# HenryHZY/VL-PET

Measured on AMD Instinct MI355X. Metric: multitask samples/sec (BART-base, r=96), higher is better.
Workload: dtype bf16

## Files before the change

vl-pet_amd/csrc/attn.hip:

```cpp
#include <cstdlib>
#include "common.h"
#include "kernels.h"
#include "attn_common.h"

#define AT_NW 4

__device__ __forceinline__ void stage_image(uint8_t* img, const __bf16* src, int64_t rs, int n_rows, int rows_pad, int tid, int nthreads) {
    const u32x4 z = {0u, 0u, 0u, 0u};
    for (int idx = tid; idx < rows_pad * 8; idx += nthreads) {
        const int row = idx >> 3, pc = idx & 7;
        u32x4 v = z;
        if (row < n_rows) v = __builtin_nontemporal_load(reinterpret_cast<const u32x4*>(src + (int64_t)row * rs + pc * 8));
        *reinterpret_cast<u32x4*>(img + (size_t)row * AT_ROW + pc * 16) = v;
    }
}
template <int NIMG, int MAXP>
__device__ __forceinline__ void stage_images(uint8_t* const* img, const __bf16* const* src, const int* n_rows, const int* rows_pad,
                                             const int64_t* rs, int tid, int nthreads) {
    u32x4 v[NIMG][MAXP];
#pragma unroll
    for (int g = 0; g < NIMG; ++g)
#pragma unroll
        for (int c = 0; c < MAXP; ++c) {
            const int idx = tid + c * nthreads, row = idx >> 3, pc = idx & 7;
            const int rr = row < n_rows[g] ? row : n_rows[g] - 1;
            v[g][c] = __builtin_nontemporal_load(reinterpret_cast<const u32x4*>(src[g] + (int64_t)rr * rs[g] + pc * 8));
        }
    const u32x4 z = {0u, 0u, 0u, 0u};
#pragma unroll
    for (int g = 0; g < NIMG; ++g)
#pragma unroll
        for (int c = 0; c < MAXP; ++c) {
            const int idx = tid + c * nthreads, row = idx >> 3, pc = idx & 7;
            if (row < rows_pad[g]) *reinterpret_cast<u32x4*>(img[g] + (size_t)row * AT_ROW + pc * 16) = row < n_rows[g] ? v[g][c] : z;
        }
}

#define AT_FW 2

struct AttnLds {
    __host__ __device__ static constexpr size_t fwd_wave_bytes(int Lkp) { return (size_t)Lkp * AT_ROW + (size_t)AT_STG + (size_t)Lkp * 4; }
    static size_t fwd_bytes(int Lkp) { return (size_t)AT_FW * fwd_wave_bytes(Lkp); }
    static size_t bwd_bytes(int Lqp, int Lkp) {
        return bwd_bytes_nw(Lqp, Lkp, AT_NW);
    }
    static size_t bwd_bytes_nw(int Lqp, int Lkp, int nw) {
        return (size_t)2 * (Lqp + Lkp) * AT_ROW + (size_t)nw * AT_STG + (size_t)Lqp * 12 + (size_t)Lkp * 4;
    }
};

__device__ __forceinline__ float key_bias(const AttnArgs& a, const uint8_t* km, int key) {
    return (key < a.Lk && (km == nullptr || km[key] != 0)) ? 0.f : -INFINITY;
}

template <int T, bool BIAS>
__global__ __launch_bounds__(AT_FW * 64, (T <= 2 ? 3 : 2)) void attn_fwd_kernel(AttnArgs a) {
    extern __shared__ __attribute__((aligned(16))) uint8_t smem[];
    const int tid = threadIdx.x, lane = tid & 63, wave = __builtin_amdgcn_readfirstlane(tid >> 6);
    const int bh = blockIdx.x * AT_FW + wave;
    if (bh >= a.B * a.H) return;
    const uint64_t seed = a.thr ? vlpet_eff_seed(a.seed, a.seed_ctr) : 0;
    const int b = bh / a.H, h = bh % a.H;
    const int m = lane & 31, hh = lane >> 5;
    constexpr int Lkp = 32 * T;
    const int64_t rs = (int64_t)a.H * 64, rq = a.ld_q, rk = a.ld_kv, rv = a.ld_v;
    const __bf16* qb_ = a.q + (int64_t)b * a.Lq * rq + h * 64;
    const __bf16* kb_ = a.k + (int64_t)b * a.Lk * rk + h * 64;
    const __bf16* vb_ = a.v + (int64_t)b * a.Lk * rv + h * 64;
    __bf16* ob_ = a.o + (int64_t)b * a.Lq * rs + h * 64;
    const uint8_t* km = a.key_mask ? a.key_mask + (int64_t)b * a.Lk : nullptr;
    uint8_t* Vs = smem + (size_t)wave * AttnLds::fwd_wave_bytes(Lkp);
    uint8_t* stg = Vs + (size_t)Lkp * AT_ROW;
    float* kval = reinterpret_cast<float*>(stg + AT_STG);
#pragma unroll
    for (int c = 0; c < (Lkp + 63) / 64; ++c)
        if (lane + 64 * c < Lkp) kval[lane + 64 * c] = key_bias(a, km, lane + 64 * c);
    const int coff = a.causal ? a.Lk - a.Lq : (1 << 20);

    bf16x8 kf[T][4];
#pragma unroll
    for (int t = 0; t < T; ++t) {
        const int j = 32 * t + m, jk = j < a.Lk ? j : a.Lk - 1;
#pragma unroll
        for (int ks = 0; ks < 4; ++ks) kf[t][ks] = *reinterpret_cast<const bf16x8*>(kb_ + (int64_t)jk * rk + 16 * ks + 8 * hh);
    }
    stage_image(Vs, vb_, rv, a.Lk, Lkp, lane, 64);

    const float sc2 = a.scale * AT_LOG2E;
    const int NQB = (a.Lq + 31) >> 5;
    for (int qb = 0; qb < NQB; ++qb) {
        const int i = 32 * qb + m;
        const int iq = i < a.Lq ? i : a.Lq - 1;
        bf16x8 qf[4];
#pragma unroll
        for (int ks = 0; ks < 4; ++ks) qf[ks] = *reinterpret_cast<const bf16x8*>(qb_ + (int64_t)iq * rq + 16 * ks + 8 * hh);
        f32x16 st[T];
#pragma unroll
        for (int t = 0; t < T; ++t) {
            if constexpr (BIAS) st[t] = bias_tile(a.bias + ((int64_t)h * (32 * NQB) + i) * Lkp + 32 * t + 4 * hh, 1.0f / a.scale);
            else st[t] = zero16();
#pragma unroll
            for (int ks = 0; ks < 4; ++ks) st[t] = mfma32(kf[t][ks], qf[ks], st[t]);
        }
        float mx = -INFINITY;
        const int ic = i + coff - 4 * hh;
#pragma unroll
        for (int t = 0; t < T; ++t) {
#pragma unroll
            for (int q4 = 0; q4 < 4; ++q4) {
                const f32x4 kv = *reinterpret_cast<const f32x4*>(kval + 32 * t + 8 * q4 + 4 * hh);
#pragma unroll
                for (int e = 0; e < 4; ++e) {
                    const int r = 4 * q4 + e;
                    float s = fmaf(st[t][r], sc2, kv[e]);
                    s = 32 * t + e + 8 * q4 > ic ? -INFINITY : s;
                    st[t][r] = s;
                    mx = fmaxf(mx, s);
                }
            }
        }
        mx = fmaxf(mx, __shfl_xor(mx, 32));
        if (mx == -INFINITY) mx = 0.f;
        float sum = 0.f;
#pragma unroll
        for (int t = 0; t < T; ++t) {
#pragma unroll
            for (int r = 0; r < 16; ++r) { const float p = fast_exp2(st[t][r] - mx); st[t][r] = p; sum += p; }
        }
        sum += __shfl_xor(sum, 32);
        const float inv = sum > 0.f ? 1.0f / sum : 0.f;
        if (hh == 0 && i < a.Lq) a.lse[((int64_t)b * a.H + h) * a.Lq + i] = sum > 0.f ? mx + log2f(sum) : INFINITY;
        const uint32_t rk = row_key(seed, ((int64_t)b * a.H + h) * a.Lq + iq);
        const float inv_keep = a.thr ? a.inv_keep : 1.0f;
        f32x16 ot0 = zero16(), ot1 = zero16();
#pragma unroll
        for (int t = 0; t < T; ++t) {
            if (a.keep_out != nullptr && a.thr != 0) {
#pragma unroll
                for (int r = 0; r < 16; ++r) {
                    const int key = 32 * t + (r & 3) + 8 * (r >> 2) + 4 * hh;
                    if (i < a.Lq && key < a.Lk)
                        a.keep_out[(((int64_t)b * a.H + h) * a.Lq + i) * a.Lk + key] = keep_elem(rk, key, a.thr) ? 1 : 0;
                }
            }
            const uint32_t kg0 = rk + (uint32_t)(32 * t + 4 * hh) * AT_GOLD;
#pragma unroll
            for (int r = 0; r < 16; ++r) {
                const int ir = (r & 3) + 8 * (r >> 2);
                const bool kp = hash_elem(kg0 + (uint32_t)ir * AT_GOLD) >= a.thr;
                st[t][r] = kp ? st[t][r] * inv * inv_keep : 0.f;
            }
#pragma unroll
            for (int u = 0; u < 2; ++u) {
                const bf16x8 pf = acc_frag(st[t], u);
                ot0 = mfma32(tr_acc_order(Vs, 32 * t + 16 * u, 0, lane), pf, ot0);
                ot1 = mfma32(tr_acc_order(Vs, 32 * t + 16 * u, 32, lane), pf, ot1);
            }
        }
        store_rows_T(stg, ot0, ot1, ob_, rs, 32 * qb, a.Lq, lane);
    }
}

enum { IMG_Q = 0, IMG_D = 1, IMG_K = 2, IMG_V = 3 };
struct BwdCtx {
    const float* rowt;
    const float* kval;
    int Lqp;
    float sc2, scale, inv_keep;
    uint32_t thr;
    int coff;
};
__device__ __forceinline__ BwdCtx bwd_ctx(const AttnArgs& a, const float* rowt, const float* kval, int Lqp) {
    BwdCtx c;
    c.rowt = rowt; c.kval = kval; c.Lqp = Lqp;
    c.sc2 = a.scale * AT_LOG2E; c.scale = a.scale; c.inv_keep = a.thr ? a.inv_keep : 1.0f; c.thr = a.thr;
    c.coff = a.causal ? a.Lk - a.Lq : (1 << 20);
    return c;
}

template <class R, bool BIAS>
__device__ __forceinline__ void bwd_k_unit(const AttnArgs& a, const BwdCtx& c, const R& rd0, int t, int NQB, int Lqp, int Lkp, int h, int lane,
                                           f32x16& dv0, f32x16& dv1, f32x16& dk0, f32x16& dk1) {
    const int m = lane & 31, hh = lane >> 5;
    const int key = 32 * t + m;
    const float kb = c.kval[key];
    const uint32_t kg = (uint32_t)key * AT_GOLD;
    const int kc = key - c.coff - 4 * hh;
    for (int qb = 0; qb < NQB; ++qb) {
        const R rd = rd0.fresh();
        f32x16 s, dp = zero16();
        if constexpr (BIAS) s = bias_tile(a.bias_t + ((int64_t)h * Lkp + key) * Lqp + 32 * qb + 4 * hh, 1.0f / a.scale);
        else s = zero16();
#pragma unroll
        for (int ks = 0; ks < 4; ++ks) {
            s = mfma32(rd.nat(IMG_Q, qb, ks), rd.nat(IMG_K, t, ks), s);
            dp = mfma32(rd.nat(IMG_D, qb, ks), rd.nat(IMG_V, t, ks), dp);
        }
        const int kcq = kc - 32 * qb;
        const float* rtp = c.rowt + 32 * qb + 4 * hh;
#pragma unroll
        for (int q4 = 0; q4 < 4; ++q4) {
            __builtin_amdgcn_sched_barrier(0);
            const f32x4 ls = *reinterpret_cast<const f32x4*>(rtp + 8 * q4);
            const f32x4 dl = *reinterpret_cast<const f32x4*>(rtp + c.Lqp + 8 * q4);
            const f32x4 rk = *reinterpret_cast<const f32x4*>(rtp + 2 * c.Lqp + 8 * q4);
#pragma unroll
            for (int e = 0; e < 4; ++e) {
                const int r = 4 * q4 + e, ir = e + 8 * q4;
                float x = fmaf(s[r], c.sc2, kb - ls[e]);
                x = kcq > ir ? -INFINITY : x;
                const float p = fast_exp2(x);
                const bool kp = hash_elem(__float_as_uint(rk[e]) + kg) >= c.thr;
                const float g = kp ? dp[r] * c.inv_keep : 0.f;
                s[r] = kp ? p * c.inv_keep : 0.f;
                dp[r] = p * (g - dl[e]) * c.scale;
            }
        }
#pragma unroll
        for (int u = 0; u < 2; ++u) {
            const bf16x8 pf = acc_frag(s, u), sf = acc_frag(dp, u);
            dv0 = mfma32(rd.tr(IMG_D, 2 * qb + u, 0), pf, dv0);
            dv1 = mfma32(rd.tr(IMG_D, 2 * qb + u, 1), pf, dv1);
            dk0 = mfma32(rd.tr(IMG_Q, 2 * qb + u, 0), sf, dk0);
            dk1 = mfma32(rd.tr(IMG_Q, 2 * qb + u, 1), sf, dk1);
        }
    }
}
template <class R, bool BIAS>
__device__ __forceinline__ void bwd_q_unit(const AttnArgs& a, const BwdCtx& c, const R& rd0, int qb, int T, int Lqp, int Lkp, int h, int lane,
                                           f32x16& dq0, f32x16& dq1) {
    const int m = lane & 31, hh = lane >> 5;
    const int i = 32 * qb + m;
    bf16x8 qf[4], df[4];
#pragma unroll
    for (int ks = 0; ks < 4; ++ks) { qf[ks] = rd0.nat(IMG_Q, qb, ks); df[ks] = rd0.nat(IMG_D, qb, ks); }
    const float l2 = c.rowt[i], dl = c.rowt[c.Lqp + i];
    const uint32_t rkey = __float_as_uint(c.rowt[2 * c.Lqp + i]);
    const int ic = i + c.coff - 4 * hh;
    for (int t = 0; t < T; ++t) {
        const R rd = rd0.fresh();
        f32x16 s, dp = zero16();
        if constexpr (BIAS) s = bias_tile(a.bias + ((int64_t)h * Lqp + i) * Lkp + 32 * t + 4 * hh, 1.0f / a.scale);
        else s = zero16();
#pragma unroll
        for (int ks = 0; ks < 4; ++ks) {
            s = mfma32(rd.nat(IMG_K, t, ks), qf[ks], s);
            dp = mfma32(rd.nat(IMG_V, t, ks), df[ks], dp);
        }
        const float* kvp = c.kval + 32 * t + 4 * hh;
        const uint32_t kg0 = rkey + (uint32_t)(32 * t + 4 * hh) * AT_GOLD;
        const int ict = ic - 32 * t;
#pragma unroll
        for (int q4 = 0; q4 < 4; ++q4) {
            __builtin_amdgcn_sched_barrier(0);
            const f32x4 kv = *reinterpret_cast<const f32x4*>(kvp + 8 * q4);
#pragma unroll
            for (int e = 0; e < 4; ++e) {
                const int r = 4 * q4 + e, ir = e + 8 * q4;
                float x = fmaf(s[r], c.sc2, kv[e] - l2);
                x = ir > ict ? -INFINITY : x;
                const float p = fast_exp2(x);
                const bool kp = hash_elem(kg0 + (uint32_t)ir * AT_GOLD) >= c.thr;
                const float g = kp ? dp[r] * c.inv_keep : 0.f;
                dp[r] = p * (g - dl) * c.scale;
            }
        }
#pragma unroll
        for (int u = 0; u < 2; ++u) {
            const bf16x8 sf = acc_frag(dp, u);
            dq0 = mfma32(rd.tr(IMG_K, 2 * t + u, 0), sf, dq0);
            dq1 = mfma32(rd.tr(IMG_K, 2 * t + u, 1), sf, dq1);
        }
    }
}
struct PadRd {
    const uint8_t* img[4];
    int m, hh, lane;
    __device__ __forceinline__ PadRd fresh() const { PadRd r = *this; asm volatile("" : "+v"(r.m), "+v"(r.lane)); return r; }
    __device__ __forceinline__ bf16x8 nat(int im, int tile, int ks) const { return nat_frag(img[im], 32 * tile + m, ks, hh); }
    __device__ __forceinline__ bf16x8 tr(int im, int g16, int dt) const { return tr_acc_order(img[im], 16 * g16, 32 * dt, lane); }
};
template <int OCC, int NW = AT_NW, bool BIAS = false>
__global__ __launch_bounds__(NW * 64, OCC) void attn_bwd_kernel(AttnArgs a) {
    extern __shared__ __attribute__((aligned(16))) uint8_t smem[];
    const int bh = blockIdx.x, b = bh / a.H, h = bh % a.H;
    const int tid = threadIdx.x, lane = tid & 63, wave = __builtin_amdgcn_readfirstlane(tid >> 6);
    const uint64_t seed = a.thr ? vlpet_eff_seed(a.seed, a.seed_ctr) : 0;
    const int m = lane & 31, hh = lane >> 5;
    const int Lkp = (a.Lk + 31) & ~31, T = Lkp >> 5;
    const int Lqp = (a.Lq + 31) & ~31, NQB = Lqp >> 5;
    const int64_t rs = (int64_t)a.H * 64, rq = a.ld_q, rk = a.ld_kv, rv = a.ld_v;
    const int64_t ooff = (int64_t)b * a.Lq * rs + h * 64;
    const int64_t qoff = (int64_t)b * a.Lq * rq + h * 64, koff = (int64_t)b * a.Lk * rk + h * 64;
    const int64_t voff = (int64_t)b * a.Lk * rv + h * 64;
    const uint8_t* km = a.key_mask ? a.key_mask + (int64_t)b * a.Lk : nullptr;
    uint8_t* Qs = smem;
    uint8_t* Ds = Qs + (size_t)Lqp * AT_ROW;
    uint8_t* Ks = Ds + (size_t)Lqp * AT_ROW;
    uint8_t* Vs = Ks + (size_t)Lkp * AT_ROW;
    uint8_t* stg = Vs + (size_t)Lkp * AT_ROW + (size_t)wave * AT_STG;
    float* rowt = reinterpret_cast<float*>(Vs + (size_t)Lkp * AT_ROW + (size_t)NW * AT_STG);
    float* kval = rowt + 3 * Lqp;

    {
        bf16x8 xo[2][2], xd[2][2];
#pragma unroll
        for (int c = 0; c < 2; ++c) {
            const int idx = tid + c * NW * 64, row = idx >> 2, part = idx & 3;
            const int rr = row < a.Lq ? row : a.Lq - 1;
#pragma unroll
            for (int e = 0; e < 2; ++e) {
                xo[c][e] = __builtin_nontemporal_load(reinterpret_cast<const bf16x8*>(a.o + ooff + (int64_t)rr * rs + 16 * part + 8 * e));
                xd[c][e] = __builtin_nontemporal_load(reinterpret_cast<const bf16x8*>(a.dout + ooff + (int64_t)rr * rs + 16 * part + 8 * e));
            }
        }
        if (tid < Lkp) kval[tid] = key_bias(a, km, tid);
        uint8_t* const imgs[4] = {Qs, Ds, Ks, Vs};
        const __bf16* const srcs[4] = {a.q + qoff, a.dout + ooff, a.k + koff, a.v + voff};
        const int nr[4] = {a.Lq, a.Lq, a.Lk, a.Lk}, rp[4] = {Lqp, Lqp, Lkp, Lkp};
        const int64_t rss[4] = {rq, rs, rk, rv};
        stage_images<4, (NW == 6 ? 3 : 4)>(imgs, srcs, nr, rp, rss, tid, NW * 64);
#pragma unroll
        for (int c = 0; c < 2; ++c) {
            const int idx = tid + c * NW * 64, row = idx >> 2, part = idx & 3;
            float acc = 0.f;
#pragma unroll
            for (int e = 0; e < 2; ++e)
#pragma unroll
                for (int j = 0; j < 8; ++j) acc += (float)xo[c][e][j] * (float)xd[c][e][j];
            acc += __shfl_xor(acc, 1);
            acc += __shfl_xor(acc, 2);
            if (part == 0 && row < Lqp) {
                const bool live = row < a.Lq;
                rowt[row] = live ? a.lse[((int64_t)b * a.H + h) * a.Lq + row] : INFINITY;
                rowt[Lqp + row] = live ? acc : 0.f;
                rowt[2 * Lqp + row] = __uint_as_float(row_key(seed, ((int64_t)b * a.H + h) * a.Lq + (live ? row : a.Lq - 1)));
            }
        }
    }
    __syncthreads();

    const BwdCtx c = bwd_ctx(a, rowt, kval, Lqp);
    PadRd rd;
    rd.img[IMG_Q] = Qs; rd.img[IMG_D] = Ds; rd.img[IMG_K] = Ks; rd.img[IMG_V] = Vs;
    rd.m = m; rd.hh = hh; rd.lane = lane;
    for (int un = (a.dbg & 1) ? T + NQB : wave; un < T + NQB; un += NW) {
        if (un < T) {
            f32x16 dv0 = zero16(), dv1 = zero16(), dk0 = zero16(), dk1 = zero16();
            if (!(a.dbg & 8)) bwd_k_unit<PadRd, BIAS>(a, c, rd, un, NQB, Lqp, Lkp, h, lane, dv0, dv1, dk0, dk1);
            if (a.dbg & 4) { if (dv0[0] + dv1[1] + dk0[2] + dk1[3] == 1.2345f) a.dv[0] = (__bf16)1.f; continue; }
            store_rows_T(stg, dv0, dv1, a.dv + voff, rv, 32 * un, a.Lk, lane);
            store_rows_T(stg, dk0, dk1, a.dk + koff, rk, 32 * un, a.Lk, lane);
        } else {
            f32x16 dq0 = zero16(), dq1 = zero16();
            if (!(a.dbg & 8)) bwd_q_unit<PadRd, BIAS>(a, c, rd, un - T, T, Lqp, Lkp, h, lane, dq0, dq1);
            if (a.dbg & 4) { if (dq0[0] + dq1[1] == 1.2345f) a.dq[0] = (__bf16)1.f; continue; }
            store_rows_T(stg, dq0, dq1, a.dq + qoff, rq, 32 * (un - T), a.Lq, lane);
        }
    }
}

size_t attn_lds_bytes(int Lq, int Lk, int bwd) {
    const int Lqp = (Lq + 31) & ~31, Lkp = (Lk + 31) & ~31;
    return bwd ? AttnLds::bwd_bytes(Lqp, Lkp) : AttnLds::fwd_bytes(Lkp);
}

template <int T, bool BIAS>
static hipError_t launch_attn_fwd_tb(const AttnArgs& a, hipStream_t stream) {
    const size_t lds = AttnLds::fwd_bytes(32 * T);
    auto kern = attn_fwd_kernel<T, BIAS>;
    hipError_t e = hipFuncSetAttribute(reinterpret_cast<const void*>(kern), hipFuncAttributeMaxDynamicSharedMemorySize, (int)lds);
    if (e != hipSuccess) return e;
    const unsigned pairs = (unsigned)(a.B * a.H);
    hipLaunchKernelGGL(kern, dim3((pairs + AT_FW - 1) / AT_FW), dim3(AT_FW * 64), lds, stream, a);
    return hipGetLastError();
}

template <int T>
static hipError_t launch_attn_fwd_t(const AttnArgs& a, hipStream_t stream) {
    return a.bias != nullptr ? launch_attn_fwd_tb<T, true>(a, stream) : launch_attn_fwd_tb<T, false>(a, stream);
}

hipError_t launch_attn(const AttnArgs& a_in, bool bwd, hipStream_t stream) {
    AttnArgs a = a_in;
    a.dbg = VLPET_IS_DEBUG_BUILD ? vlpet_tuning().dbg : 0;
    if (!bwd) {
        switch ((a.Lk + 31) >> 5) {
            case 1: return launch_attn_fwd_t<1>(a, stream);
            case 2: return launch_attn_fwd_t<2>(a, stream);
            case 3: return launch_attn_fwd_t<3>(a, stream);
            case 4: return launch_attn_fwd_t<4>(a, stream);
            default: return hipErrorInvalidValue;
        }
    }
    const int Lqp = (a.Lq + 31) & ~31, Lkp = (a.Lk + 31) & ~31;
    const int units = (Lqp >> 5) + (Lkp >> 5);
    const int occ_env = vlpet_tuning().attn_occ;
    const int nw_env = vlpet_tuning().attn_nw;
    const size_t lds6 = AttnLds::bwd_bytes_nw(Lqp, Lkp, 6);
    if (nw_env == 6 && (units == 5 || units == 6) && 2 * (lds6 + 512) <= (size_t)160 * 1024) {
        auto k6 = attn_bwd_kernel<3, 6>;
        hipError_t e6 = hipFuncSetAttribute(reinterpret_cast<const void*>(k6), hipFuncAttributeMaxDynamicSharedMemorySize, (int)lds6);
        if (e6 != hipSuccess) return e6;
        hipLaunchKernelGGL(k6, dim3((unsigned)(a.B * a.H)), dim3(6 * 64), lds6, stream, a);
        return hipGetLastError();
    }
    const size_t lds = attn_lds_bytes(a.Lq, a.Lk, 1);
    if (a.bias != nullptr) {
        const bool o3 = occ_env == 3 || (occ_env != 2 && 3 * (lds + 512) <= (size_t)160 * 1024);
        const void* kb = o3 ? reinterpret_cast<const void*>(attn_bwd_kernel<3, AT_NW, true>) : reinterpret_cast<const void*>(attn_bwd_kernel<2, AT_NW, true>);
        hipError_t eb = hipFuncSetAttribute(kb, hipFuncAttributeMaxDynamicSharedMemorySize, (int)lds);
        if (eb != hipSuccess) return eb;
        if (o3) hipLaunchKernelGGL((attn_bwd_kernel<3, AT_NW, true>), dim3((unsigned)(a.B * a.H)), dim3(AT_NW * 64), lds, stream, a);
        else hipLaunchKernelGGL((attn_bwd_kernel<2, AT_NW, true>), dim3((unsigned)(a.B * a.H)), dim3(AT_NW * 64), lds, stream, a);
        return hipGetLastError();
    }
    const bool occ3 = occ_env == 3 || (occ_env != 2 && 3 * (lds + 512) <= (size_t)160 * 1024);
    const void* kern = occ3 ? reinterpret_cast<const void*>(attn_bwd_kernel<3>) : reinterpret_cast<const void*>(attn_bwd_kernel<2>);
    hipError_t e = hipFuncSetAttribute(kern, hipFuncAttributeMaxDynamicSharedMemorySize, (int)lds);
    if (e != hipSuccess) return e;
    if (occ3) hipLaunchKernelGGL(attn_bwd_kernel<3>, dim3((unsigned)(a.B * a.H)), dim3(AT_NW * 64), lds, stream, a);
    else hipLaunchKernelGGL(attn_bwd_kernel<2>, dim3((unsigned)(a.B * a.H)), dim3(AT_NW * 64), lds, stream, a);
    return hipGetLastError();
}
```

vl-pet_amd/csrc/kernels.h:

```cpp
#pragma once
#include <cstdlib>
#include <hip/hip_runtime.h>
#include <stdint.h>
#include "rng.h"
#include "tuning.h"

#define VLPET_MAX_HEADS 16

struct PackArgs {
    const void* wd[VLPET_MAX_HEADS];
    const void* bd[VLPET_MAX_HEADS];
    const void* wu;
    const void* bu;
    int n_heads, rows_per_head;
    int r, d, RT;
    int src_bf16;
    int n_packs;
    uint8_t* out;
};
hipError_t launch_pack_pair(const PackArgs& a, int NS, hipStream_t stream);
#define VLPET_PACK_BATCH 8
struct PackBatch { PackArgs p[VLPET_PACK_BATCH]; int n; };
hipError_t launch_pack_pairs(const PackBatch& b, int NS, hipStream_t stream);

#define PET_GATE 1
#define PET_GATE_ADD 2
#define PET_ACT_IDENTITY 4

struct PetFwdArgs {
    const void* xa;
    const void* res;
    const void* xg;
    void* out;
    const uint8_t* pk_a;
    const uint8_t* pk_g;
    DropSpec drop;
    int64_t M;
    int d, RT;
    float s2, sd, gs;
    int flags;
    void* save;
    int64_t save_stride;
    int dbg;
    unsigned long long* dbg_ts;
    int d_in;
    const uint8_t* pk_a_dn;
    const uint8_t* pk_g_dn;
    float gm, go;
};
hipError_t launch_pet_fwd(const PetFwdArgs& a, int io_fp32, hipStream_t stream);
hipError_t launch_pet_gate_fwd(const PetFwdArgs& a, int io_fp32, hipStream_t stream);
hipError_t launch_pet_lowrank_fwd(const PetFwdArgs& a, int io_fp32, hipStream_t stream);
bool k1_fwd2p_applies(const PetFwdArgs& a, int io_fp32);
bool k1_fwd2p_preferred(const PetFwdArgs& a);
hipError_t launch_k1_fwd2p(const PetFwdArgs& a, int passes, hipStream_t stream);

struct PetBwdArgs {
    const void* dy;
    const void* xa;
    const void* res;
    const void* xg;
    void* dxa;
    void* dxg;
    const void* dxg_in;
    void* z_a; void* dp_a;
    void* z_g; void* dp_g;
    void* dh; void* dq;
    const uint8_t* pk_a;
    const uint8_t* pk_g;
    DropSpec drop;
    const void* saved;
    int64_t saved_stride;
    int64_t M;
    int d, RT;
    float s2, sd, gs;
    int flags;
    float gm, go;
    int fsplit;
    float* dz_part;
    const void* y;
    unsigned* red_ctrl;
    int red_words;
};
hipError_t launch_pet_bwd(const PetBwdArgs& a, int io_fp32, hipStream_t stream);
bool pet_gate_bwd2_applies(const PetBwdArgs& a);
hipError_t launch_pet_gate_bwd2(const PetBwdArgs& a, int io_fp32, hipStream_t stream);
hipError_t launch_pet_lowrank_bwd(const PetBwdArgs& a, int io_fp32, hipStream_t stream);

struct WgradJob {
    const void* P; int ldp; int pcols;
    const void* X; int ldx; int xcols;
    DropSpec drop; int has_drop;
    float scale;
    float* out; int ldo; int transposed;
    int out_rows;
    float* colsum_x;
    float* colsum_p;
};
struct WgradArgs {
    WgradJob job[4];
    int njobs;
    int64_t M;
    int RT;
    int row_chunks;
    int64_t rows_per_chunk;
    float* partial;
    int nslice;
};
struct WgradLayout {
    int64_t off[4];
    int64_t total;
};
__host__ __device__ inline WgradLayout wgrad_layout(const WgradArgs& a) {
    WgradLayout L;
    int64_t o = 0;
    const int PR = 32 * a.RT;
    for (int j = 0; j < 4; ++j) {
        L.off[j] = o;
        if (j < a.njobs) o += (int64_t)a.row_chunks * ((int64_t)PR * a.job[j].xcols + a.job[j].xcols + PR);
    }
    L.total = o;
    return L;
}
size_t wgrad_workspace_bytes(int njobs, int RT, int xcols_max, int row_chunks);
hipError_t launch_wgrad_finalize(const WgradArgs& a, hipStream_t stream);
void wgrad_plan(int64_t M, int njobs, int xcols_max, int* row_chunks, int64_t* rows_per_chunk);
hipError_t launch_wgrad(const WgradArgs& a, int io_fp32, hipStream_t stream);
bool ng_two_pass_applies(const PetBwdArgs& a, int io_fp32);
void ng_cols_plan(int64_t M, int d, int* row_chunks, int64_t* rows_per_chunk);
hipError_t launch_ng_two_pass(const PetBwdArgs& b, const WgradArgs& g, int passes, hipStream_t stream);
bool k4_wgrad2_applies(int64_t M, int F, int d_out, int io_fp32);
size_t k4_wgrad2_workspace_bytes(int64_t M, int F, int d_out);
hipError_t launch_k4_wgrad2(const void* dpre, const void* feats, float* dw, float* db, void* workspace, int64_t M, int F, int d_out,
                            hipStream_t stream);

bool pet_gate_bwd3_applies(const PetBwdArgs& a);
void gate_bwd3_plan(int64_t M, int d, int io_fp32, int* row_chunks, int64_t* rows_per_chunk, int* GS, int* NG);
hipError_t launch_pet_gate_dz(const PetBwdArgs& a, int io_fp32, hipStream_t stream);
bool k1_dz2_applies(const PetBwdArgs& a, int io_fp32);
hipError_t launch_k1_dz2(const PetBwdArgs& a, hipStream_t stream);
int k1_dz2_feature_blocks(int64_t M, int d);
bool k1_dz6_applies(const PetBwdArgs& a, int io_fp32);
hipError_t launch_k1_dz6(const PetBwdArgs& a, hipStream_t stream);
int k1_dz6_feature_blocks(int64_t M, int d);
hipError_t launch_k1_dz_reduce(const PetBwdArgs& a, int PR, hipStream_t stream);
hipError_t launch_pet_gate_cols(const PetBwdArgs& a, const WgradArgs& g, int GS, int NG, int io_fp32, hipStream_t stream);

struct ColsRedJob {
    float* out; int ldo, transposed, out_rows; float scale;
    float* colsum_x;
    float* colsum_p;
};
struct ColsRedArgs {
    float* slab;
    float* bias_x;
    float* bias_p;
    unsigned* ctrl;
    ColsRedJob job[4];
    unsigned spin_limit;
};
#define COLS_RED_STRIDE 320
#define COLS_RED_SPIN_DEFAULT (1u << 13)
struct ColzArgs {
    const void* dy; const void* x1; const void* x2;
    const void* dxin;
    const void* y;
    const void* z_a; const void* z_g;
    const void* dp_a; const void* dp_g;
    void* dx1; void* dx2;
    const uint8_t* pk_a; const uint8_t* pk_g;
    int64_t M;
    int d;
    float s2, sd, gs;
    int flags;
    int row_chunks; int64_t rows_per_chunk;
    float* part[4];
    ColsRedArgs red;
};
void k1_cols_plan(int64_t M, int d, int* row_chunks, int64_t* rows_per_chunk);
bool k1_cols_applies(const PetBwdArgs& a, int io_fp32);
hipError_t launch_k1_cols(const ColzArgs& c, int RT, hipStream_t stream);
void k1_cols6_plan(int64_t M, int d, int* row_chunks, int64_t* rows_per_chunk);
bool k1_cols6_applies(const PetBwdArgs& a, int io_fp32);
hipError_t launch_k1_cols6y(const ColzArgs& c, hipStream_t stream);

struct VisprojArgs {
    const void* feats;
    const uint8_t* pk;
    const float* gamma;
    const float* beta;
    const void* R;
    void* out;
    void* xhat;
    float* rstd;
    int64_t M;
    int F, d_out;
    float eps;
    int rms;
};
hipError_t launch_visproj_fwd(const VisprojArgs& a, int io_fp32, hipStream_t stream);

struct VisGemmArgs {
    const void* feats; const void* w;
    const float* bias; const float* gamma; const float* beta;
    const void* R; void* out; void* xhat; float* rstd; float* mean;
    unsigned long long* xch;
    unsigned* status;
    unsigned* flags;
    unsigned long long* stats;
    unsigned spin_limit;
    int64_t M; int F, d_out; float eps; int rms;
    int nteams, row_blocks;
};

bool visproj_gemm_applies(int64_t M, int F, int d_out, int io_fp32);
size_t visproj_gemm_workspace_bytes(int64_t M, int F, int d_out);
size_t visproj_gemm_exchange_bytes(int d_out);
hipError_t launch_visproj_gemm(VisGemmArgs& a, void* ws, int form, int bm, hipStream_t stream);

struct VisPosArgs {
    const float* pos;
    const float* w; const float* b;
    const float* gamma; const float* beta;
    const void* img_tab; const void* obj_tab;
    int img_tab_bf16, obj_tab_bf16;
    const int64_t* img_ids; const int64_t* obj_ids;
    int64_t img_bstride, obj_bstride;
    int n_img; int64_t obj_rows;
    void* out;
    const void* dout;
    float* partial;
    float* dw; float* db; float* dgamma; float* dbeta; float* dimg;
    int64_t M; int N, d; float eps; int rms;
};
bool vispos_applies(int d, int n_img);
size_t vispos_bwd_workspace_bytes(int64_t M, int d, int n_img);
hipError_t launch_vispos_fwd(const VisPosArgs& a, int io_fp32, hipStream_t stream);
hipError_t launch_vispos_bwd(const VisPosArgs& a, int io_fp32, hipStream_t stream);

struct TailArgs {
    const void* y;
    const void* x1;
    void* out;
    void* h;
    const float* gamma;
    const float* beta;
    float* mean;
    float* rstd;
    uint8_t* keep_out;
    float* dgb;
    int64_t M;
    int d;
    float eps;
    uint32_t thr;
    float keep_scale;
    uint64_t seed;
    const uint64_t* seed_ctr;
    int norm;
    int post;
    int h_xhat;
    int h_out;
    const void* dres;
    int rms;
    void* out2;
    const float* gamma2;
};
hipError_t launch_tail(const TailArgs& a, int io_fp32, bool bwd, hipStream_t stream);
int tail_blocks(int64_t M);

struct Lora8Args {
    const void* x; const void* base; void* out;
    const uint8_t* pk;
    DropSpec drop;
    void* save;
    int64_t M; int d;
    float scaling;
};
bool lora8_applies(int64_t M, int d, int r, int io_fp32);
hipError_t launch_lora8_fwd(const Lora8Args& a, hipStream_t stream);
hipError_t launch_tail_reduce(const float* part, int nb, int d, float* dgamma, float* dbeta, hipStream_t stream);
hipError_t launch_colsum(const void* x, int64_t M, int n, float* part, float* out, int io_fp32, hipStream_t stream);
hipError_t launch_colsum_partial(const void* x, int64_t M, int n, float* part, int io_fp32, hipStream_t stream);
struct ReduceJob { const float* part; float* out0; float* out1; int nb; int d; };
#define VLPET_REDUCE_BATCH 96
struct ReduceBatch { ReduceJob j[VLPET_REDUCE_BATCH]; int n; };
hipError_t launch_tail_reduce_batch(const ReduceBatch& b, int max_d, hipStream_t stream);

struct PoolArgs {
    const void* x;
    void* out;
    int64_t n_img;
    int s_in, s_out, dim;
};
hipError_t launch_downsample(const PoolArgs& a, int in_fp32, int out_fp32, hipStream_t stream);

enum RowOp { ROW_DOT = 0, ROW_AFFINE = 1, ROW_BWD = 2, VEC_FWD = 3, VEC_BWD = 4 };
struct RowArgs {
    const void* a;
    const void* c;
    const void* e;
    void* o1;
    void* o2;
    const float* va;
    const float* vc;
    const float* ra;
    const float* rb;
    float* rs;
    float* part;
    int64_t M;
    int d;
};
hipError_t launch_rowgate(const RowArgs& a, int op, int io_fp32, hipStream_t stream);
int rowgate_blocks(int64_t M);

struct AdamwArgs {
    float* p; float* g; float* m; float* v;
    const uint8_t* decay;
    int64_t n;
    const float* partials; int n_partials;
    float max_norm;
    float grad_scale;
    float lr, beta1, beta2, eps, weight_decay;
    float bias_c1, bias_c2_sqrt;
    int decay_first;
    int eps_scaled;
    int zero_grad;
    float* norm_out;
    const int32_t* slice_of;
    const float* slice_bc;
};
hipError_t launch_add_inplace(void* dst, const void* src, int64_t n, int io_fp32, hipStream_t stream);
struct SumNArgs { const void* src[8]; void* out; };
hipError_t launch_sum_n(const SumNArgs& a, int n, int64_t len, int io_fp32, hipStream_t stream);
hipError_t launch_sumsq(const float* g, int64_t n, float* partials, hipStream_t stream);
hipError_t launch_adamw(const AdamwArgs& a, hipStream_t stream);
int optim_blocks(int64_t n);

inline int pick_row_groups(int64_t M, int max_rg, int min_rg) {
    if (const int rg = vlpet_tuning().rg; rg >= min_rg && rg <= max_rg && rg > 0) return rg;
    int best = max_rg;
    int64_t best_cost = -1;
    for (int rg = max_rg; rg >= min_rg; --rg) {
        const int64_t wgs = (M + 32 * rg - 1) / (32 * rg);
        const int64_t cost = ((wgs + 255) / 256) * (rg + 1);
        if (best_cost < 0 || cost < best_cost) { best = rg; best_cost = cost; }
    }
    return best;
}

#define VLPET_ACT_GELU 0
#define VLPET_ACT_GELU_NEW 1
#define VLPET_ACT_RELU 2
struct ActDropArgs {
    const void* x;
    const void* dy;
    void* out;
    uint8_t* keep_out;
    int64_t n;
    int act;
    uint32_t thr;
    float keep_scale;
    uint64_t seed;
    const uint64_t* seed_ctr;
};
hipError_t launch_act_dropout(const ActDropArgs& a, bool bwd, int io_fp32, hipStream_t stream);
hipError_t launch_cat_dropout(const void* a, const void* v, void* x, int64_t B, int La, int Lv, int d, uint32_t thr, float keep_scale,
                              uint64_t seed, const uint64_t* seed_ctr, bool bwd, int io_fp32, hipStream_t stream);

struct CeArgs {
    const void* logits;
    const int64_t* labels;
    float* loss;
    float* lse;
    const float* dloss;
    void* dlogits;
    int64_t N;
    int V, ld;
    unsigned int* bad;
};
hipError_t launch_ce(const CeArgs& a, bool bwd, int io_fp32, hipStream_t stream);

struct AttnArgs {
    const __bf16* q; const __bf16* k; const __bf16* v;
    __bf16* o;
    float* lse;
    const __bf16* dout;
    __bf16* dq; __bf16* dk; __bf16* dv;
    const uint8_t* key_mask;
    const float* bias;
    const float* bias_t;
    uint8_t* keep_out;
    int B, H, Lq, Lk, causal;
    int ld_q, ld_kv;
    int ld_v;
    float scale;
    uint32_t thr;
    float inv_keep;
    uint64_t seed;
    const uint64_t* seed_ctr;
    int dbg;
};
size_t attn_lds_bytes(int Lq, int Lk, int bwd);
hipError_t launch_attn(const AttnArgs& a, bool bwd, hipStream_t stream);
hipError_t launch_attn_long_fwd(const AttnArgs& a, hipStream_t stream);
hipError_t launch_attn_long_bwd(const AttnArgs& a, float* delta, hipStream_t stream);

struct AdapterTailArgs {
    const void* h;
    const void* res;
    const void* wd;
    const void* bd;
    const void* wu;
    const void* bu;
    const float* gamma;
    const float* beta;
    void* out;
    int64_t M;
    int d, r;
    float scale, eps;
    int norm;
};
int adapter_tail_rows(void);
bool adapter_tail_geometry_ok(int d, int r);
hipError_t launch_adapter_tail(const AdapterTailArgs& a, int io_fp32, int param_fp32, hipStream_t stream);

struct PhmLayer {
    const void* rule;
    const void* W;
    void* wt;
    const float* dwt;
    float* drule;
    float* dW;
    int in, out;
};
struct PhmArgs {
    PhmLayer l[2];
    int n;
    float* ws;
};
int64_t phm_layer_tiles(int in, int out, int n);
hipError_t launch_phm_expand_fwd(const PhmArgs& a, int param_fp32, hipStream_t stream);
hipError_t launch_phm_expand_bwd(const PhmArgs& a, int param_fp32, hipStream_t stream);
```

vl-pet_amd/csrc/tuning.h:

```cpp
#pragma once
#include <cstdlib>

struct VlpetTuning {
    int rg = 0;
    int bwd2 = 1;
    int bwd3 = -1;
    int bwd3_units = 0;
    int bwd3_form = 1;
    int k4_waves4 = 0;
    int wgrad_wgs = 0;
    int wgrad_tr = 1;
    int wgrad_stream = 1;
    int wgrad_nstg = 3;
    int wgs_mode = 0;
    int attn_occ = 0;
    int attn_nw = 0;
    int dz2 = 1;
    int dz2_fsplit = 0;
    int dz6 = 1;
    int k4_wgrad2 = 1;
    int ng2 = 1;
    int fwd2p = -1;
    int cols_red = 1;
    int dbg = 0;
};

#ifdef VLPET_DEBUG
inline const VlpetTuning& vlpet_tuning() {
    static const VlpetTuning t = [] {
        VlpetTuning v;
        auto rd = [](const char* n, int& dst) { if (const char* e = getenv(n)) dst = atoi(e); };
        rd("VLPET_RG", v.rg); rd("VLPET_BWD2", v.bwd2); rd("VLPET_BWD3", v.bwd3); rd("VLPET_BWD3_UNITS", v.bwd3_units);
        rd("VLPET_BWD3_FORM", v.bwd3_form); rd("VLPET_K4_WAVES4", v.k4_waves4); rd("VLPET_WGRAD_WGS", v.wgrad_wgs);
        rd("VLPET_WGRAD_TR", v.wgrad_tr); rd("VLPET_WGRAD_STREAM", v.wgrad_stream); rd("VLPET_WGRAD_NSTG", v.wgrad_nstg);
        rd("VLPET_WGS_MODE", v.wgs_mode); rd("VLPET_ATTN_OCC", v.attn_occ); rd("VLPET_ATTN_NW", v.attn_nw); rd("VLPET_DBG", v.dbg); rd("VLPET_DZ2", v.dz2); rd("VLPET_DZ6", v.dz6); rd("VLPET_DZ2_FSPLIT", v.dz2_fsplit); rd("VLPET_K4_WGRAD2", v.k4_wgrad2); rd("VLPET_NG2", v.ng2); rd("VLPET_FWD2P", v.fwd2p); rd("VLPET_COLS_RED", v.cols_red);
        return v;
    }();
    return t;
}
#define VLPET_IS_DEBUG_BUILD 1
#else
inline const VlpetTuning& vlpet_tuning() { static const VlpetTuning t{}; return t; }
#define VLPET_IS_DEBUG_BUILD 0
#endif
```

Before: 29500.

## Add single-wave-per-head attention backward kernel for short query lengths

Adds a dedicated attention backward kernel for Lq<=32 without bias, where each wave handles one batch-head pair and streams K/V tiles with register prefetch. dS is transposed through LDS using ds_read_tr, with an alternative recompute path available in debug builds. It is enabled by default and targets decoder or short-query cases, where the general block kernel wastes work and occupancy on padded query tiles. The risk is lower parallelism per head and a possible load imbalance when there are few batch-head pairs.

```diff
diff --git a/vl-pet_amd/csrc/attn.hip b/vl-pet_amd/csrc/attn.hip
--- a/vl-pet_amd/csrc/attn.hip
+++ b/vl-pet_amd/csrc/attn.hip
@@ -393,6 +393,7 @@
             default: return hipErrorInvalidValue;
         }
     }
+    if (a.Lq <= 32 && a.bias == nullptr && vlpet_tuning().attn_fewq != 0) return launch_attn_bwd_fewq(a, stream);
     const int Lqp = (a.Lq + 31) & ~31, Lkp = (a.Lk + 31) & ~31;
     const int units = (Lqp >> 5) + (Lkp >> 5);
     const int occ_env = vlpet_tuning().attn_occ;
diff --git a/vl-pet_amd/csrc/attn_bwd_fewq.hip b/vl-pet_amd/csrc/attn_bwd_fewq.hip
--- /dev/null
+++ b/vl-pet_amd/csrc/attn_bwd_fewq.hip
@@ -0,0 +1,247 @@
+#include "common.h"
+#include "kernels.h"
+#include "attn_common.h"
+#include "tuning.h"
+
+#define AT_FQ 4
+#define AT_DS_ROW 72
+
+struct FewqLds {
+    static constexpr size_t IMG = (size_t)32 * AT_ROW;
+    static constexpr size_t Q = 0, D = IMG, K = 2 * IMG, DS = 3 * IMG, STG = DS + 32 * AT_DS_ROW;
+    static constexpr size_t ROWT = STG + AT_STG;
+    static constexpr size_t KVAL = ROWT + 3 * 32 * 4;
+    static constexpr size_t wave_bytes = KVAL + 128 * 4;
+    static constexpr size_t bytes = AT_FQ * wave_bytes;
+};
+static_assert(FewqLds::wave_bytes % 16 == 0 && FewqLds::STG % 16 == 0 && FewqLds::ROWT % 16 == 0, "16-byte aligned LDS sections");
+static_assert(2 * (FewqLds::bytes + 512) <= (size_t)160 * 1024, "two workgroups per CU");
+
+__device__ __forceinline__ bf16x8 tr_ds_tile(const uint8_t* img, int kb, int lane) {
+    const int g = lane >> 4, sl = lane & 15;
+    const uint8_t* p = img + (size_t)(kb + 4 * (g >> 1) + (sl >> 2)) * AT_DS_ROW + (16 * (g & 1) + 4 * (sl & 3)) * 2;
+    typedef __attribute__((address_space(3))) v4s16_t lds_v4;
+    const v4s16_t lo = __builtin_amdgcn_ds_read_tr16_b64_v4i16((lds_v4*)(p));
+    const v4s16_t hi = __builtin_amdgcn_ds_read_tr16_b64_v4i16((lds_v4*)(p + 8 * AT_DS_ROW));
+    const v8s16_t r = {lo[0], lo[1], lo[2], lo[3], hi[0], hi[1], hi[2], hi[3]};
+    return __builtin_bit_cast(bf16x8, r);
+}
+
+struct FewqTile { u32x4 kx[4]; bf16x8 vf[4]; };
+__device__ __forceinline__ void fewq_load_tile(FewqTile& r, const __bf16* kb_, const __bf16* vb_, int64_t rk, int64_t rv, int t, int Lk, int lane) {
+    const int m = lane & 31, hh = lane >> 5;
+#pragma unroll
+    for (int c = 0; c < 4; ++c) {
+        const int idx = lane + 64 * c, row = 32 * t + (idx >> 3), pc = idx & 7;
+        const int rr = row < Lk ? row : Lk - 1;
+        r.kx[c] = __builtin_nontemporal_load(reinterpret_cast<const u32x4*>(kb_ + (int64_t)rr * rk + pc * 8));
+    }
+    const int j = 32 * t + m, jv = j < Lk ? j : Lk - 1;
+#pragma unroll
+    for (int ks = 0; ks < 4; ++ks) r.vf[ks] = __builtin_nontemporal_load(reinterpret_cast<const bf16x8*>(vb_ + (int64_t)jv * rv + 16 * ks + 8 * hh));
+}
+
+__device__ __forceinline__ void fewq_put_tile(uint8_t* Kt, bf16x8 (&vf)[4], const FewqTile& r, int t, int Lk, int lane) {
+    const u32x4 z = {0u, 0u, 0u, 0u};
+#pragma unroll
+    for (int c = 0; c < 4; ++c) {
+        const int idx = lane + 64 * c, row = idx >> 3, pc = idx & 7;
+        *reinterpret_cast<u32x4*>(Kt + (size_t)row * AT_ROW + pc * 16) = 32 * t + row < Lk ? r.kx[c] : z;
+    }
+#pragma unroll
+    for (int ks = 0; ks < 4; ++ks) vf[ks] = r.vf[ks];
+}
+
+template <bool TWICE>
+__global__ __launch_bounds__(AT_FQ * 64, 2) void attn_bwd_fewq_kernel(AttnArgs a) {
+    extern __shared__ __attribute__((aligned(16))) uint8_t smem[];
+    const int tid = threadIdx.x, lane = tid & 63, wave = __builtin_amdgcn_readfirstlane(tid >> 6);
+    const int bh = blockIdx.x * AT_FQ + wave;
+    if (bh >= a.B * a.H) return;
+    const uint64_t seed = a.thr ? vlpet_eff_seed(a.seed, a.seed_ctr) : 0;
+    const int b = bh / a.H, h = bh % a.H;
+    const int m = lane & 31, hh = lane >> 5;
+    const int T = (a.Lk + 31) >> 5;
+    const int64_t rs = (int64_t)a.H * 64, rq = a.ld_q, rk = a.ld_kv, rv = a.ld_v;
+    const int64_t ooff = (int64_t)b * a.Lq * rs + h * 64;
+    const int64_t qoff = (int64_t)b * a.Lq * rq + h * 64, koff = (int64_t)b * a.Lk * rk + h * 64;
+    const int64_t voff = (int64_t)b * a.Lk * rv + h * 64;
+    uint8_t* base = smem + (size_t)wave * FewqLds::wave_bytes;
+    uint8_t* Qs = base + FewqLds::Q;
+    uint8_t* Ds = base + FewqLds::D;
+    uint8_t* Kt = base + FewqLds::K;
+    uint8_t* dsT = base + FewqLds::DS;
+    uint8_t* stg = base + FewqLds::STG;
+    float* rowt = reinterpret_cast<float*>(base + FewqLds::ROWT);
+    float* kval = reinterpret_cast<float*>(base + FewqLds::KVAL);
+    const u32x4 z = {0u, 0u, 0u, 0u};
+
+    FewqTile nx;
+    bf16x8 vf[4];
+    {
+        const bool live_m = m < a.Lq;
+        const float lse_m = a.lse[((int64_t)b * a.H + h) * a.Lq + (live_m ? m : a.Lq - 1)];
+        uint8_t kmv[2] = {1, 1};
+        if (a.key_mask != nullptr) {
+#pragma unroll
+            for (int c = 0; c < 2; ++c) {
+                const int key = lane + 64 * c;
+                kmv[c] = a.key_mask[(int64_t)b * a.Lk + (key < a.Lk ? key : a.Lk - 1)];
+            }
+        }
+        u32x4 xq[4], xd[4], xo[4];
+#pragma unroll
+        for (int c = 0; c < 4; ++c) {
+            const int idx = lane + 64 * c, row = idx >> 3, pc = idx & 7;
+            const int rr = row < a.Lq ? row : a.Lq - 1;
+            xq[c] = __builtin_nontemporal_load(reinterpret_cast<const u32x4*>(a.q + qoff + (int64_t)rr * rq + pc * 8));
+            xd[c] = __builtin_nontemporal_load(reinterpret_cast<const u32x4*>(a.dout + ooff + (int64_t)rr * rs + pc * 8));
+            xo[c] = __builtin_nontemporal_load(reinterpret_cast<const u32x4*>(a.o + ooff + (int64_t)rr * rs + pc * 8));
+        }
+        fewq_load_tile(nx, a.k + koff, a.v + voff, rk, rv, 0, a.Lk, lane);
+        if (hh == 0) {
+            rowt[m] = live_m ? lse_m : INFINITY;
+            rowt[64 + m] = __uint_as_float(row_key(seed, ((int64_t)b * a.H + h) * a.Lq + (live_m ? m : a.Lq - 1)));
+        }
+#pragma unroll
+        for (int c = 0; c < 2; ++c) {
+            const int key = lane + 64 * c;
+            kval[key] = (key < a.Lk && kmv[c] != 0) ? 0.f : -INFINITY;
+        }
+#pragma unroll
+        for (int c = 0; c < 4; ++c) {
+            const int idx = lane + 64 * c, row = idx >> 3, pc = idx & 7;
+            const bool live = row < a.Lq;
+            *reinterpret_cast<u32x4*>(Qs + (size_t)row * AT_ROW + pc * 16) = live ? xq[c] : z;
+            *reinterpret_cast<u32x4*>(Ds + (size_t)row * AT_ROW + pc * 16) = live ? xd[c] : z;
+            const bf16x8 fo = __builtin_bit_cast(bf16x8, xo[c]), fd = __builtin_bit_cast(bf16x8, xd[c]);
+            float acc = 0.f;
+#pragma unroll
+            for (int j = 0; j < 8; ++j) acc += (float)fo[j] * (float)fd[j];
+            float acc2 = __shfl_xor(acc, 1);
+#pragma unroll
+            for (int j = 0; j < 8; ++j) acc2 += (float)fo[j] * (float)fd[j];
+            acc2 += __shfl_xor(acc2, 2);
+            acc2 += __shfl_xor(acc2, 4);
+            if (pc == 1) rowt[32 + row] = live ? acc2 : 0.f;
+        }
+    }
+    fewq_put_tile(Kt, vf, nx, 0, a.Lk, lane);
+    const float sc2 = a.scale * AT_LOG2E, scale = a.scale, inv_keep = a.thr ? a.inv_keep : 1.0f;
+    const uint32_t thr = a.thr;
+    const int coff = a.causal ? a.Lk - a.Lq : (1 << 20);
+
+    f32x16 dq0 = zero16(), dq1 = zero16();
+    for (int t = 0; t < T; ++t) {
+        asm volatile("" ::: "memory");
+        if (t + 1 < T) fewq_load_tile(nx, a.k + koff, a.v + voff, rk, rv, t + 1, a.Lk, lane);
+
+        const int key = 32 * t + m;
+        const float kb = kval[key];
+        const uint32_t kg = (uint32_t)key * AT_GOLD;
+        const int kc = key - coff - 4 * hh;
+        f32x16 s = zero16(), dp = zero16();
+#pragma unroll
+        for (int ks = 0; ks < 4; ++ks) {
+            s = mfma32(nat_frag(Qs, m, ks, hh), nat_frag(Kt, m, ks, hh), s);
+            dp = mfma32(nat_frag(Ds, m, ks, hh), vf[ks], dp);
+        }
+        const float* rtp = rowt + 4 * hh;
+#pragma unroll
+        for (int q4 = 0; q4 < 4; ++q4) {
+            const f32x4 ls = *reinterpret_cast<const f32x4*>(rtp + 8 * q4);
+            const f32x4 dl = *reinterpret_cast<const f32x4*>(rtp + 32 + 8 * q4);
+            const f32x4 rkq = *reinterpret_cast<const f32x4*>(rtp + 64 + 8 * q4);
+#pragma unroll
+            for (int e = 0; e < 4; ++e) {
+                const int r = 4 * q4 + e, ir = e + 8 * q4;
+                float x = fmaf(s[r], sc2, kb - ls[e]);
+                x = kc > ir ? -INFINITY : x;
+                const float p = fast_exp2(x);
+                const bool kp = hash_elem(__float_as_uint(rkq[e]) + kg) >= thr;
+                const float g = kp ? dp[r] * inv_keep : 0.f;
+                s[r] = kp ? p * inv_keep : 0.f;
+                dp[r] = p * (g - dl[e]) * scale;
+            }
+        }
+        f32x16 dv0 = zero16(), dv1 = zero16(), dk0 = zero16(), dk1 = zero16();
+        bf16x8 sf[2];
+#pragma unroll
+        for (int u = 0; u < 2; ++u) {
+            const bf16x8 pf = acc_frag(s, u);
+            sf[u] = acc_frag(dp, u);
+            dv0 = mfma32(tr_acc_order(Ds, 16 * u, 0, lane), pf, dv0);
+            dv1 = mfma32(tr_acc_order(Ds, 16 * u, 32, lane), pf, dv1);
+            dk0 = mfma32(tr_acc_order(Qs, 16 * u, 0, lane), sf[u], dk0);
+            dk1 = mfma32(tr_acc_order(Qs, 16 * u, 32, lane), sf[u], dk1);
+        }
+        bf16x8 qf[2];
+        if constexpr (!TWICE) {
+            typedef __bf16 bf16x4_t __attribute__((ext_vector_type(4)));
+#pragma unroll
+            for (int g = 0; g < 4; ++g) {
+                const bf16x4_t w = {sf[g >> 1][4 * (g & 1)], sf[g >> 1][4 * (g & 1) + 1], sf[g >> 1][4 * (g & 1) + 2], sf[g >> 1][4 * (g & 1) + 3]};
+                *reinterpret_cast<bf16x4_t*>(dsT + (size_t)m * AT_DS_ROW + (8 * g + 4 * hh) * 2) = w;
+            }
+            asm volatile("" ::: "memory");
+#pragma unroll
+            for (int u = 0; u < 2; ++u) qf[u] = tr_ds_tile(dsT, 16 * u, lane);
+        } else {
+            f32x16 s2 = zero16(), dp2 = zero16();
+#pragma unroll
+            for (int ks = 0; ks < 4; ++ks) {
+                s2 = mfma32(nat_frag(Kt, m, ks, hh), nat_frag(Qs, m, ks, hh), s2);
+                dp2 = mfma32(vf[ks], nat_frag(Ds, m, ks, hh), dp2);
+            }
+            const float l2 = rowt[m], dl2 = rowt[32 + m];
+            const uint32_t kg0 = __float_as_uint(rowt[64 + m]) + (uint32_t)(32 * t + 4 * hh) * AT_GOLD;
+            const int ict = m + coff - 4 * hh - 32 * t;
+            const float* kvp = kval + 32 * t + 4 * hh;
+#pragma unroll
+            for (int q4 = 0; q4 < 4; ++q4) {
+                const f32x4 kv = *reinterpret_cast<const f32x4*>(kvp + 8 * q4);
+#pragma unroll
+                for (int e = 0; e < 4; ++e) {
+                    const int r = 4 * q4 + e, ir = e + 8 * q4;
+                    float x = fmaf(s2[r], sc2, kv[e] - l2);
+                    x = ir > ict ? -INFINITY : x;
+                    const float p = fast_exp2(x);
+                    const bool kp = hash_elem(kg0 + (uint32_t)ir * AT_GOLD) >= thr;
+                    const float g = kp ? dp2[r] * inv_keep : 0.f;
+                    dp2[r] = p * (g - dl2) * scale;
+                }
+            }
+#pragma unroll
+            for (int u = 0; u < 2; ++u) qf[u] = acc_frag(dp2, u);
+        }
+#pragma unroll
+        for (int u = 0; u < 2; ++u) {
+            dq0 = mfma32(tr_acc_order(Kt, 16 * u, 0, lane), qf[u], dq0);
+            dq1 = mfma32(tr_acc_order(Kt, 16 * u, 32, lane), qf[u], dq1);
+        }
+        asm volatile("" ::: "memory");
+        if (t + 1 < T) fewq_put_tile(Kt, vf, nx, t + 1, a.Lk, lane);
+        asm volatile("" ::: "memory");
+        store_rows_T(stg, dv0, dv1, a.dv + voff, rv, 32 * t, a.Lk, lane);
+        store_rows_T(stg, dk0, dk1, a.dk + koff, rk, 32 * t, a.Lk, lane);
+    }
+    store_rows_T(stg, dq0, dq1, a.dq + qoff, rq, 0, a.Lq, lane);
+}
+
+template <bool TWICE>
+static hipError_t launch_fewq(const AttnArgs& a, hipStream_t stream) {
+    auto kern = attn_bwd_fewq_kernel<TWICE>;
+    hipError_t e = hipFuncSetAttribute(reinterpret_cast<const void*>(kern), hipFuncAttributeMaxDynamicSharedMemorySize, (int)FewqLds::bytes);
+    if (e != hipSuccess) return e;
+    const unsigned pairs = (unsigned)(a.B * a.H);
+    hipLaunchKernelGGL(kern, dim3((pairs + AT_FQ - 1) / AT_FQ), dim3(AT_FQ * 64), FewqLds::bytes, stream, a);
+    return hipGetLastError();
+}
+
+hipError_t launch_attn_bwd_fewq(const AttnArgs& a, hipStream_t stream) {
+    if (a.Lq > 32 || a.Lk > 128 || a.bias != nullptr) return hipErrorInvalidValue;
+#if VLPET_IS_DEBUG_BUILD
+    if (vlpet_tuning().attn_fewq == 2) return launch_fewq<true>(a, stream);
+#endif
+    return launch_fewq<false>(a, stream);
+}
diff --git a/vl-pet_amd/csrc/kernels.h b/vl-pet_amd/csrc/kernels.h
--- a/vl-pet_amd/csrc/kernels.h
+++ b/vl-pet_amd/csrc/kernels.h
@@ -402,6 +402,7 @@
 };
 size_t attn_lds_bytes(int Lq, int Lk, int bwd);
 hipError_t launch_attn(const AttnArgs& a, bool bwd, hipStream_t stream);
+hipError_t launch_attn_bwd_fewq(const AttnArgs& a, hipStream_t stream);
 hipError_t launch_attn_long_fwd(const AttnArgs& a, hipStream_t stream);
 hipError_t launch_attn_long_bwd(const AttnArgs& a, float* delta, hipStream_t stream);
 
diff --git a/vl-pet_amd/csrc/tuning.h b/vl-pet_amd/csrc/tuning.h
--- a/vl-pet_amd/csrc/tuning.h
+++ b/vl-pet_amd/csrc/tuning.h
@@ -15,6 +15,7 @@
     int wgs_mode = 0;
     int attn_occ = 0;
     int attn_nw = 0;
+    int attn_fewq = 1;
     int dz2 = 1;
     int dz2_fsplit = 0;
     int dz6 = 1;
@@ -33,7 +34,7 @@
         rd("VLPET_RG", v.rg); rd("VLPET_BWD2", v.bwd2); rd("VLPET_BWD3", v.bwd3); rd("VLPET_BWD3_UNITS", v.bwd3_units);
         rd("VLPET_BWD3_FORM", v.bwd3_form); rd("VLPET_K4_WAVES4", v.k4_waves4); rd("VLPET_WGRAD_WGS", v.wgrad_wgs);
         rd("VLPET_WGRAD_TR", v.wgrad_tr); rd("VLPET_WGRAD_STREAM", v.wgrad_stream); rd("VLPET_WGRAD_NSTG", v.wgrad_nstg);
-        rd("VLPET_WGS_MODE", v.wgs_mode); rd("VLPET_ATTN_OCC", v.attn_occ); rd("VLPET_ATTN_NW", v.attn_nw); rd("VLPET_DBG", v.dbg); rd("VLPET_DZ2", v.dz2); rd("VLPET_DZ6", v.dz6); rd("VLPET_DZ2_FSPLIT", v.dz2_fsplit); rd("VLPET_K4_WGRAD2", v.k4_wgrad2); rd("VLPET_NG2", v.ng2); rd("VLPET_FWD2P", v.fwd2p); rd("VLPET_COLS_RED", v.cols_red);
+        rd("VLPET_WGS_MODE", v.wgs_mode); rd("VLPET_ATTN_OCC", v.attn_occ); rd("VLPET_ATTN_NW", v.attn_nw); rd("VLPET_ATTN_FEWQ", v.attn_fewq); rd("VLPET_DBG", v.dbg); rd("VLPET_DZ2", v.dz2); rd("VLPET_DZ6", v.dz6); rd("VLPET_DZ2_FSPLIT", v.dz2_fsplit); rd("VLPET_K4_WGRAD2", v.k4_wgrad2); rd("VLPET_NG2", v.ng2); rd("VLPET_FWD2P", v.fwd2p); rd("VLPET_COLS_RED", v.cols_red);
         return v;
     }();
     return t;
```

New measurement: 29880, median of 6. 1.3% higher.
